# lcp29/trimesh-ray-optix

Hardware: AMD Instinct MI355X
Metric: Mrays/s closest-hit, 1M-tri mesh, 1024^2 ray batch (higher is better)
Workload: dtype f32; 1 GPU; C5(i): icosphere(8)+displacement seed 0, 1310720 tris; 1024x1024 pinhole rays per GPU; intersects_closest (stream_compaction=False); rays_per_gpu=1048576, rays_total=1048576, triangles=1310720, parallelism=ray-sharded x1, BVH replicated, warmup_steps_done=328, bvh_depth=30, bvh_bytes=104857568

## Files before the change

### trimesh-ray-optix_amd/csrc/kernels_direct.inc

```
template <bool C, bool DEEP = false> struct tr_word { typedef uint64_t T; };
template <> struct tr_word<true, false> { typedef uint32_t T; };

constexpr bool TR_STREAM_QN = true;
template <int Q> constexpr bool TR_STREAM_COLD = Q != TR_Q_CLOSEST;
template <int Q, int K, bool STATS, bool COMPACT = false, bool UNI = false, bool DEEP = false>
__device__ __forceinline__ void wave_traverse(const tr_bvh_view& b, tr_ray& r, bool go,
                                              tr_result& res, tr_topk<K>& top, tr_counters* cnt,
                                              const tr_ring ring) {
    tr_result_init(res);
    if (Q == TR_Q_LOCATION) top.init();
    typedef typename tr_word<COMPACT, DEEP>::T W;
    tr_state_t<W> fs;
    tr_state_init(fs);
    if (!go) fs.node = -1;
    while (!tr_done(fs)) {
        tr_fused_step<Q, K, STATS, COMPACT, W, UNI, true>(b, r, fs, res, top, cnt, ring);
        TR_CONVERGE();
        tr_fused_step<Q, K, STATS, COMPACT, W, UNI, false>(b, r, fs, res, top, cnt, ring);
        TR_CONVERGE();
    }
}

constexpr uint32_t TR_STEAL_EVERY = 3u;
constexpr uint32_t TR_STEAL_EARLY = 4u;
constexpr int TR_STEAL_IDLE = 1;
__device__ __forceinline__ int lane_rank(unsigned long long mask) {
    return (int)__builtin_amdgcn_mbcnt_hi((unsigned)(mask >> 32), __builtin_amdgcn_mbcnt_lo((unsigned)mask, 0u));
}

template <int Q, bool STATS, bool COMPACT, bool DEEP = false, bool QN = false>
__device__ __forceinline__ bool wave_traverse_steal(const tr_bvh_view& b, tr_ray& r, bool go,
                                                    tr_result& res, tr_counters* cnt,
                                                    const tr_ring ring, int32_t* wl, int lane,
                                                    uint32_t steal_min) {
    typedef typename tr_word<COMPACT, DEEP>::T W;
    tr_result_init(res);
    tr_topk<1> top;
    tr_state_t<W> fs;
    tr_state_init(fs);
    if (!go) fs.node = -1;
    auto trip_step = [&](auto test_tag) {
        constexpr bool TEST = decltype(test_tag)::value;
        if (!tr_done(fs)) tr_fused_step<Q, 1, STATS, COMPACT, W, false, TEST, QN>(b, r, fs, res, top, cnt, ring);
    };
    int owner = lane;
    bool split = false;
    uint32_t trip = 0;
    if (steal_min & 0x8000u) {
        steal_min &= 0x7fffu;
        const unsigned long long act = __ballot(go);
        if (act != 0ull) {
            const int l0 = (int)__builtin_ctzll(act);
            const float ax = __shfl(r.dx, l0), ay = __shfl(r.dy, l0), az = __shfl(r.dz, l0);
            const float bx = __shfl(r.ox, l0) - r.ox, by = __shfl(r.oy, l0) - r.oy, bz = __shfl(r.oz, l0) - r.oz;
            const float dd = ax * r.dx + ay * r.dy + az * r.dz;
            const float n0 = ax * ax + ay * ay + az * az, n1 = r.dx * r.dx + r.dy * r.dy + r.dz * r.dz;
            const float ex = 65535.f * b.frame.scale[0], ey = 65535.f * b.frame.scale[1], ez = 65535.f * b.frame.scale[2];
            const bool alike = dd > 0.f && dd * dd >= 0.998f * n0 * n1 && bx * bx + by * by + bz * bz <= 1e-4f * (ex * ex + ey * ey + ez * ez);
            if (4 * __popcll(__ballot(go && alike)) < 3 * __popcll(act) && steal_min > TR_STEAL_EARLY) steal_min = TR_STEAL_EARLY;
        }
    }
    typedef __attribute__((address_space(3))) volatile int32_t lds_i32;
    typedef __attribute__((address_space(3))) volatile unsigned long long lds_u64;
    lds_i32* const lw = (lds_i32*)wl;
    lds_i32* const list = lw;
    lds_i32* const xnode = lw + 64;
    lds_i32* const xdepth = lw + 128;
    constexpr int ACC = 192;
    int32_t* sum = wl + ACC;
    unsigned long long* keys = reinterpret_cast<unsigned long long*>(wl + ACC);
    lds_i32* const vsum = lw + ACC;
    lds_u64* const vkeys = (lds_u64*)(lw + ACC);
    lds_i32* const vslots = lw + ACC + 128;
    auto deposit = [&]() {
        if (Q == TR_Q_COUNT) {
            if (res.count) atomicAdd(&sum[owner], res.count);
        } else if (Q == TR_Q_ANY) {
            if (res.best_face >= 0) vsum[owner] = 1;
        } else {
            const bool have = res.best_slot >= 0;
            const unsigned long long key = ((unsigned long long)(__float_as_uint(res.best_t) & 0x7fffffffu) << 32) |
                                           (unsigned)res.best_face;
            if (have) atomicMin(&keys[owner], key);
            __builtin_amdgcn_wave_barrier();
            if (have && vkeys[owner] == key) vslots[owner] = res.best_slot;
        }
    };
    for (;;) {
#pragma unroll 1
        for (uint32_t k = 0; k <= TR_STEAL_EVERY; k += 2) {
            trip_step(std::true_type{});
            TR_CONVERGE();
            trip_step(std::false_type{});
            TR_CONVERGE();
        }
        trip += (TR_STEAL_EVERY / 2u + 1u) * 2u;
        if (split) {
            if (Q == TR_Q_ANY) {
                if (res.best_face >= 0) vsum[owner] = 1;
                __builtin_amdgcn_wave_barrier();
                if (vsum[owner] != 0 && !tr_done(fs)) { fs.node = -1; fs.p0 = -1; fs.p1 = -1; fs.p2 = -1; }
            } else if (Q == TR_Q_CLOSEST || Q == TR_Q_FIRST) {
                const bool have = res.best_slot >= 0;
                const unsigned long long mine = ((unsigned long long)(__float_as_uint(res.best_t) & 0x7fffffffu) << 32) |
                                                (unsigned)(res.best_face < 0 ? 0x7fffffff : res.best_face);
                if (have) atomicMin(&keys[owner], mine);
                __builtin_amdgcn_wave_barrier();
                const unsigned long long k = vkeys[owner];
                if (have && k == mine) vslots[owner] = res.best_slot;
                if (k < mine) {
                    tr_set_best_t(res, __uint_as_float((unsigned)(k >> 32)));
                    res.best_face = (int32_t)(unsigned)k;
                    res.best_slot = -1;
                }
            }
        }
        const bool done = tr_done(fs);
        const unsigned long long idle = __ballot(done);
        if (idle == ~0ull) break;
        if (__popcll(idle) >= TR_STEAL_IDLE) {
            const W cand = fs.trail & fs.owned;
            const bool can_give = !done && cand != 0 && trip >= steal_min;
            const unsigned long long donors = __ballot(can_give);
            const int ni = __popcll(idle), nd = __popcll(donors);
            const int np = ni < nd ? ni : nd;
            if (np > 0) {
                if (!split) {
                    if (Q == TR_Q_COUNT || Q == TR_Q_ANY) vsum[lane] = 0;
                    else vkeys[lane] = ~0ull;
                    split = true;
                    __builtin_amdgcn_wave_barrier();
                }
                const int drank = lane_rank(donors), irank = lane_rank(idle);
                const bool give = can_give && drank < np;
                int gnode = 0, gdepth = 0;
                if (give) {
                    uint32_t j;
                    gnode = tr_ring_get(ring, tr_bottom_slot<W>(fs.trail, fs.owned, j));
                    gdepth = (int32_t)(j + 1);
                    list[drank] = lane; xnode[lane] = gnode; xdepth[lane] = gdepth;
                    fs.trail &= ~(W(1) << j);
                }
                __builtin_amdgcn_wave_barrier();
                const bool take = done && irank < np;
                const int src = take ? list[irank] : lane;
                if (take) {
                    deposit();
                    tr_result_init(res);
                }
                r.ox = __shfl(r.ox, src); r.oy = __shfl(r.oy, src); r.oz = __shfl(r.oz, src);
                r.dx = __shfl(r.dx, src); r.dy = __shfl(r.dy, src); r.dz = __shfl(r.dz, src);
                r.ix = __shfl(r.ix, src); r.iy = __shfl(r.iy, src); r.iz = __shfl(r.iz, src);
                r.kd = __shfl(r.kd, src);
                r.sel_n = (uint32_t)__shfl((int)r.sel_n, src); r.sel_f = (uint32_t)__shfl((int)r.sel_f, src); r.sel_z = (uint32_t)__shfl((int)r.sel_z, src);
                if constexpr (QN) {
                    r.qax = __shfl(r.qax, src); r.qay = __shfl(r.qay, src); r.qaz = __shfl(r.qaz, src);
                    r.qnx = __shfl(r.qnx, src); r.qny = __shfl(r.qny, src); r.qnz = __shfl(r.qnz, src);
                    r.qfx = __shfl(r.qfx, src); r.qfy = __shfl(r.qfy, src); r.qfz = __shfl(r.qfz, src);
                    r.qaz2 = r.qaz;
                }
                const int own2 = __shfl(owner, src);
                const float bt = __shfl(res.best_t, src);
                if (take) {
                    owner = own2;
                    tr_state_init(fs);
                    fs.node = xnode[src];
                    fs.depth = (uint32_t)xdepth[src];
                    tr_set_best_t(res, bt);
                }
                __builtin_amdgcn_wave_barrier();
            }
        }
    }
    if (split) {
        deposit();
        __builtin_amdgcn_wave_barrier();
        if (Q == TR_Q_COUNT) {
            res.count = vsum[lane];
        } else if (Q == TR_Q_ANY) {
            res.best_face = vsum[lane] ? 0 : -1;
        } else {
            const unsigned long long k = vkeys[lane];
            tr_result_init(res);
            if (k != ~0ull) {
                tr_set_best_t(res, __uint_as_float((unsigned)(k >> 32)));
                res.best_face = (int32_t)(unsigned)k;
                res.best_slot = vslots[lane];
            }
        }
    }
    return split;
}

template <int Q, bool STATS, bool COMPACT = false, bool UNI = false, bool DEEP = false>
__device__ __forceinline__ void process_ray(const tr_bvh_view& b, const RayFetch& rf,
                                            const QueryOut& out, int64_t i, bool in_range,
                                            tr_counters* cnt, const tr_ring ring) {
    float o[3] = {0.f, 0.f, 0.f}, d[3] = {0.f, 0.f, 0.f};
    if (in_range) fetch_ray(rf, i, o, d);
    tr_ray r;
    const bool valid = tr_ray_setup_a(r, b.frame, o[0], o[1], o[2], d[0], d[1], d[2]) && in_range;
    tr_result res;
    if (Q == TR_Q_LOCATION) {
        tr_topk<0> top;
        top.ent = out.hits + (in_range ? i : 0) * out.cap;
        top.tris = b.tris;
        top.cap = out.cap;
        if (b.num_tris >= 2) {
            wave_traverse<Q, 0, STATS, COMPACT, UNI, DEEP>(b, r, valid, res, top, cnt, ring);
        } else {
            top.init();
            brute_one<Q>(b, r, valid, res);
            if (res.count) top.insert(res.best_t, res.best_face, 0);
        }
    } else {
        tr_topk<1> top;
        if (b.num_tris >= 2) wave_traverse<Q, 1, STATS, COMPACT, UNI, DEEP>(b, r, valid, res, top, cnt, ring);
        else brute_one<Q>(b, r, valid, res);
    }
    if (in_range) write_result<Q>(b, out, i, r, res);
}

template <int Q, bool STATS, bool COMPACT, bool DEEP = false, bool QN = false>
__device__ __forceinline__ void process_ray_steal(const tr_bvh_view& b, const RayFetch& rf,
                                                  const QueryOut& out, int64_t i, bool in_range,
                                                  tr_counters* cnt, const tr_ring ring, int32_t* wl,
                                                  uint32_t steal_min) {
    float o[3] = {0.f, 0.f, 0.f}, d[3] = {0.f, 0.f, 0.f};
    if (in_range) fetch_ray(rf, i, o, d);
    tr_ray r;
    const bool valid = tr_ray_setup_q(r, b.frame, o[0], o[1], o[2], d[0], d[1], d[2]) && in_range;
    tr_result res;
    bool split = false;
    if (b.num_tris >= 2) split = wave_traverse_steal<Q, STATS, COMPACT, DEEP, QN>(b, r, valid, res, cnt, ring, wl, (int)(threadIdx.x & 63), steal_min);
    else brute_one<Q>(b, r, valid, res);
    if (split && in_range) {
        fetch_ray(rf, i, o, d);
        tr_ray_setup_a(r, b.frame, o[0], o[1], o[2], d[0], d[1], d[2]);
    }
    if (in_range) write_result<Q>(b, out, i, r, res);
}

template <int Q, int K, bool STATS, bool COMPACT, bool DEEP = false>
__device__ __forceinline__ void wave_traverse_unordered(const tr_bvh_view& b, tr_ray& r, bool go,
                                                        tr_result& res, tr_topk<K>& top, tr_counters* cnt,
                                                        const tr_ring ring, const tr_leafq lq, int leaf_min) {
    typedef typename tr_word<COMPACT, DEEP>::T W;
    tr_result_init(res);
    if (Q == TR_Q_LOCATION) top.init();
    tr_ustate_t<W> st;
    tr_ustate_init(st);
    if (!go) st.node = -1;
    for (;;) {
        const bool can_node = tr_ucan_node(st);
        const unsigned long long mn = __ballot(can_node), ml = __ballot(st.nq > 0);
        if ((mn | ml) == 0ull) break;
        const bool parked = st.node >= 0 && !can_node;
        const bool leaf_phase = mn == 0ull || __ballot(parked) != 0ull || (int)__popcll(ml) >= (int)leaf_min;
        tr_unord_step<Q, K, STATS, COMPACT, W>(b, r, can_node, leaf_phase, st, res, top, cnt, ring, lq);
        TR_CONVERGE();
    }
}

template <int Q, bool STATS, bool COMPACT, bool DEEP = false>
__device__ __forceinline__ int wave_count_unordered_steal(const tr_bvh_view& b, tr_ray& r, bool go, tr_counters* cnt,
                                                          const tr_ring ring, const tr_leafq lq, int leaf_min,
                                                          int lane, uint32_t steal_min) {
    typedef typename tr_word<COMPACT, DEEP>::T W;
    tr_result res;
    tr_result_init(res);
    tr_topk<1> top;
    tr_ustate_t<W> st;
    tr_ustate_init(st);
    if (!go) st.node = -1;
    int owner = lane;
    int acc = 0;
    uint32_t trip = 0;
    auto hand_in = [&](bool want) {
        unsigned long long m = __ballot(want && res.count != 0);
        while (m != 0ull) {
            const int t = (int)__builtin_ctzll(m);
            const int o = __builtin_amdgcn_readlane(owner, t), c = __builtin_amdgcn_readlane(res.count, t);
            if (lane == o) acc += c;
            m &= m - 1ull;
        }
        if (want) res.count = 0;
    };
    for (;;) {
        bool live = true;
#pragma unroll 1
        for (int k = 0; k < 4 && live; k++) {
            const bool can_node = tr_ucan_node(st);
            const unsigned long long mn = __ballot(can_node), ml = __ballot(st.nq > 0);
            live = (mn | ml) != 0ull;
            if (live) {
                const bool parked = st.node >= 0 && !can_node;
                const bool leaf_phase = mn == 0ull || __ballot(parked) != 0ull || (int)__popcll(ml) >= (int)leaf_min;
                tr_unord_step<Q, 1, STATS, COMPACT, W>(b, r, can_node, leaf_phase, st, res, top, cnt, ring, lq);
            }
            TR_CONVERGE();
        }
        trip += 4;
        const bool done = tr_udone(st);
        const unsigned long long idle = __ballot(done);
        if (idle == ~0ull) break;
        if (idle == 0ull) continue;
        const W cand = st.trail & st.owned;
        const bool can_give = !done && cand != 0 && trip >= steal_min;
        const unsigned long long donors = __ballot(can_give);
        const int ni = __popcll(idle), nd = __popcll(donors);
        const int np = ni < nd ? ni : nd;
        if (np == 0) continue;
        const int drank = lane_rank(donors), irank = lane_rank(idle);
        const bool give = can_give && drank < np;
        const bool take = done && irank < np;
        const unsigned long long givers = __ballot(give);
        const int tgt = give ? drank : 63 - lane_rank(~givers);
        const int list = __builtin_amdgcn_ds_permute(tgt << 2, lane);
        const int pick = __shfl(list, irank & 63);
        const int src = take ? pick : lane;
        int gnode = 0, gdepth = 0;
// ... 145 lines not shown
        const uint32_t q = 255u - min(255u, (uint32_t)((float)cost[i] * scale));
        const int x = i < nfull ? (i / T) & 7 : i & 7;
        const uint32_t j = atomicAdd(&bins[x][q], 1u);
        const uint32_t sp = nsplit[x], q4 = sp >> 2;
        if (j < q4) {
            for (uint32_t k = 0; k < 4u; k++)
                order[(4u * j + k) * 8u + (uint32_t)x] = (uint32_t)i | (2u << 30) | (k << 28);
        } else if (j < sp) {
            const uint32_t p = 4u * q4 + 2u * (j - q4);
            order[p * 8u + (uint32_t)x] = (uint32_t)i | (1u << 30);
            order[(p + 1u) * 8u + (uint32_t)x] = (uint32_t)i | (1u << 30) | (1u << 28);
        } else {
            order[(j + sp + 2u * q4) * 8u + (uint32_t)x] = (uint32_t)i;
        }
        if (prev) prev[i] = cost[i];
        cost[i] = 0u;
    }
    if (tid == 0) { order[TR_SCHED_MAX] = (uint32_t)nblocks; order[TR_SCHED_MAX + 1] = (uint32_t)split; }
}

template <int Q, bool STATS, bool COMPACT, int BS, int MODE, bool DEEP, bool QN, bool JOB = false>
__device__ __forceinline__ void query_direct_body(const tr_bvh_view& b, const RayFetch& rf, const QueryOut& out,
                                                  int xcd_map, int scramble, int tile_w, int steal_min,
                                                  const uint32_t* __restrict__ order, int order_split,
                                                  uint32_t* __restrict__ cost,
                                                  unsigned long long* stats,
                                                  const int* __restrict__ sel,
                                                  const tr_wide_args& wa = tr_wide_args{nullptr, nullptr, 0, 0},
                                                  const tr_sort_job& job = tr_sort_job{nullptr, nullptr, nullptr, 0, 0, 0, 0, 0, 0}) {
    if (sel && *sel != 0) return;
    const unsigned slot_shift = JOB ? 8u : 0u;
    const unsigned bid = blockIdx.x - slot_shift;
    int64_t nblk = gridDim.x - slot_shift;
    const unsigned long long t_start = cost ? wall_clock64() : 0ull;
    __shared__ int32_t ring_lds[MODE == 4 ? 1 : TR_RING * BS];
    const tr_ring ring = {ring_lds + threadIdx.x, BS};
    constexpr int SCR = 384;
    __shared__ alignas(8) int32_t steal_lds[MODE == 1 ? (BS / 64) * SCR : (JOB ? 16 : 2)];
    if constexpr (JOB) {
        static_assert((MODE == 1 || MODE == 3) && BS == 128, "the sorter rides in the launches that steal");
        if (blockIdx.x < 8) {
            static_assert(sizeof(ring_lds) >= 8 * 256 * 4 && sizeof(steal_lds) >= 16 * 4, "the sorter works on the traversal's LDS");
            if (blockIdx.x == 0 && job.cost)
                sched_sort_body<BS>(job.cost, job.order, job.nblocks, job.xcd_map, job.split, job.split4, job.outlier8,
                                    job.floor_ticks, job.prev, reinterpret_cast<uint32_t(*)[256]>(ring_lds),
                                    reinterpret_cast<uint32_t*>(steal_lds));
            return;
        }
    }
    int64_t blk = bid;
    int part = 0, parts_lg = 0;
    if (order) {
        nblk -= 8 * ((int64_t)order_split + 2 * (order_split >> 2));
        const uint32_t* hdr = order + TR_SCHED_MAX;
        if (hdr[0] != (uint32_t)nblk || hdr[1] != (uint32_t)order_split) {
            order = nullptr;
            if ((int64_t)bid >= nblk) return;
        }
    }
    if (order) {
        const uint32_t e = order[bid];
        blk = e & 0x07ffffffu;
        if (blk >= nblk) return;
        parts_lg = (int)(e >> 30);
        part = (int)((e >> 28) & 3u);
        if (MODE != 1 && MODE != 3) {
            if (part) return;
            parts_lg = 0;
        }
    } else if (xcd_map > 0) {
        const int64_t T = xcd_map, span = 8 * T;
        const int64_t nfull = nblk / span * span;
        if (blk < nfull) {
            const int64_t x = blk & 7;
            int64_t k = blk >> 3;
            if (scramble > 1) k = (k * scramble) % (nfull >> 3);
            blk = ((k / T) * 8 + x) * T + (k % T);
        }
    }
    int64_t i = blk * BS + threadIdx.x;
    if (tile_w > 0) {
        const int lgh = (tile_w >> 28) & 3, lgw = 6 - lgh;
        const int64_t width = tile_w & 0x0fffffff;
        const int64_t tile = i >> 6, tpr = width >> lgw;
        const int lane = (int)(i & 63);
        const int64_t ty = tile / tpr, tx = tile - ty * tpr;
        i = ((ty << lgh) + (lane >> lgw)) * width + (tx << lgw) + (lane & ((1 << lgw) - 1));
    }
    tr_counters cnt = {0, 0, 0};
    if (MODE == 4) {
        __shared__ int32_t wstack_lds[(TR_WNODES + TR_WLEAVES) * BS];
        const bool in_range = i < rf.n;
        float o[3] = {0.f, 0.f, 0.f}, d[3] = {0.f, 0.f, 0.f};
        if (in_range) fetch_ray(rf, i, o, d);
        tr_ray r;
        const bool valid = tr_ray_setup_q(r, b.frame, o[0], o[1], o[2], d[0], d[1], d[2]) && in_range;
        tr_result res;
        if constexpr (Q == TR_Q_LOCATION) {
            tr_topk<0> top;
            top.ent = out.hits + (in_range ? i : 0) * out.cap;
            top.tris = b.tris;
            top.cap = out.cap;
            wave_traverse_wide<Q, 0, STATS, BS>(b, wa, r, valid, res, top, cnt, wstack_lds);
        } else {
            tr_topk<1> top;
            wave_traverse_wide<Q, 1, STATS, BS>(b, wa, r, valid, res, top, cnt, wstack_lds);
        }
        if (in_range) write_result<Q>(b, out, i, r, res);
    } else if (MODE == 2) {
        __shared__ int32_t leafq_lds[TR_LEAFQ * BS];
        const tr_leafq lq = {leafq_lds + threadIdx.x, BS};
        process_ray_unordered<Q, STATS, COMPACT, DEEP>(b, rf, out, i, i < rf.n, &cnt, ring, lq, steal_min);
    } else if (MODE == 3) {
        __shared__ int32_t leafq_lds[TR_LEAFQ * BS];
        const tr_leafq lq = {leafq_lds + threadIdx.x, BS};
        const bool mine = (((int)threadIdx.x ^ part) & ((1 << parts_lg) - 1)) == 0;
        const uint32_t smin = parts_lg ? ((uint32_t)steal_min >> 20) & 0xfffu : ((uint32_t)steal_min >> 8) & 0xfffu;
        process_ray_unordered<Q, STATS, COMPACT, DEEP, true>(b, rf, out, i, i < rf.n && mine, &cnt, ring, lq,
                                                            steal_min & 0xff, smin);
    } else if (MODE == 1) {
        const bool mine = (((int)threadIdx.x ^ part) & ((1 << parts_lg) - 1)) == 0;
        const uint32_t smin = parts_lg ? (uint32_t)steal_min >> 16 : (uint32_t)steal_min & 0xffffu;
        process_ray_steal<Q, STATS, COMPACT, DEEP, QN>(b, rf, out, i, i < rf.n && mine, &cnt, ring,
                                                       steal_lds + (threadIdx.x >> 6) * SCR, smin);
    } else {
        process_ray<Q, STATS, COMPACT, !STATS && BS == 128 && Q != TR_Q_LOCATION, DEEP>(b, rf, out, i, i < rf.n, &cnt, ring);
    }
    if (cost && (threadIdx.x & 63) == 0) {
        constexpr int TR_SPLIT_STICKY = 1;
        const unsigned long long dt = (wall_clock64() - t_start) << (parts_lg ? parts_lg + TR_SPLIT_STICKY : 0);
        atomicMax(&cost[blk], (uint32_t)(dt > 0x7ffffull ? 0x7ffffull : dt));
    }
    flush_stats<STATS>(cnt, stats);
}

#ifndef TR_DIRECT_WAVES
#define TR_DIRECT_WAVES 6
#endif
#if TR_DIRECT_WAVES > 0
#ifndef TR_DEEP_WAVES
#define TR_DEEP_WAVES TR_DIRECT_WAVES
#endif
#define TR_DIRECT_W ((!COMPACT || (DEEP && !QN)) ? TR_DEEP_WAVES - 1 : DEEP ? TR_DEEP_WAVES : TR_DIRECT_WAVES)
#define TR_DIRECT_OCC __attribute__((amdgpu_waves_per_eu(TR_DIRECT_W, TR_DIRECT_W)))
#else
#define TR_DIRECT_OCC
#endif
constexpr int TR_BS = 128;
template <int Q, bool STATS, bool COMPACT, int MODE = 0, bool DEEP = false, bool QN = false>
__global__ __launch_bounds__(TR_BS) TR_DIRECT_OCC void k_query_direct(tr_bvh_view b, RayFetch rf, QueryOut out,
                                                      int xcd_map, int scramble, int tile_w, int steal_min,
                                                      const uint32_t* __restrict__ order, int order_split,
                                                      uint32_t* __restrict__ cost,
                                                      unsigned long long* stats,
                                                      const int* __restrict__ sel) {
    TR_VIEW_LIVE(b);
    query_direct_body<Q, STATS, COMPACT, TR_BS, MODE, DEEP, QN>(b, rf, out, xcd_map, scramble, tile_w, steal_min, order,
                                                                order_split, cost, stats, sel);
}
#ifndef TR_COUNT_WAVES
#define TR_COUNT_WAVES 7
#endif
#if TR_COUNT_WAVES > 0
#define TR_COUNT_W ((DEEP || !COMPACT) ? 5 : TR_COUNT_WAVES)
#define TR_COUNT_OCC __attribute__((amdgpu_waves_per_eu(TR_COUNT_W, TR_COUNT_W)))
#else
#define TR_COUNT_OCC
#endif
template <bool COMPACT, bool DEEP>
__global__ __launch_bounds__(TR_BS) TR_COUNT_OCC void k_query_count_steal(tr_bvh_view b, RayFetch rf, QueryOut out,
// ... 91 lines not shown
```

### trimesh-ray-optix_amd/csrc/tr_bvh.h

```cpp
#pragma once
#include <type_traits>
#include "tr_math.h"
#include "../../include/triro_hip.h"

struct alignas(16) tr_f4 {
    float x, y, z, w;
};
struct alignas(16) tr_i4 {
    int32_t x, y, z, w;
};

struct alignas(64) tr_node {
    float box0[6];
    float box1[6];
    int32_t c0, c1;
    int32_t parent;
    int32_t sibling;
};
static_assert(sizeof(tr_node) == 64, "node must be 64 B");
TR_HD void tr_node_set_box(float* box, const float* lo, const float* hi) {
    box[0] = lo[0]; box[1] = lo[1]; box[2] = lo[2]; box[3] = hi[2]; box[4] = hi[0]; box[5] = hi[1];
}

struct alignas(8) tr_link {
// ... 278 lines not shown
#endif
                const tr_tri u = tr_load_tri<false, COMPACT>(b, pe, nc);
                if (!tr_tie_own(r.dx, r.dy, r.dz, u.ax, u.ay, u.az, u.bx, u.by, u.bz, u.cx, u.cy, u.cz, e.tie)) tt = -1.0f;
            }
            const bool hit = tt >= TR_TMIN && tt <= TR_TMAX;
            fin = tr_fold_hit<Q, K>(hit, tt, t.face, pe, res, top);
            pe = -1;
        }
    }
    return fin;
}

#define TR_RING 16
struct tr_ring {
    int32_t* base;
    int32_t stride;
};
TR_HD int32_t tr_ring_get(const tr_ring& ring, uint32_t slot) {
#if defined(__HIP_DEVICE_COMPILE__)
    typedef __attribute__((address_space(3))) int32_t tr_lds_i32;
    return ((tr_lds_i32*)ring.base)[slot * ring.stride];
#else
    return ring.base[slot * ring.stride];
#endif
}
TR_HD void tr_ring_put(const tr_ring& ring, uint32_t slot, int32_t v) {
#if defined(__HIP_DEVICE_COMPILE__)
    typedef __attribute__((address_space(3))) int32_t tr_lds_i32;
    ((tr_lds_i32*)ring.base)[slot * ring.stride] = v;
#else
    ring.base[slot * ring.stride] = v;
#endif
}

template <typename W>
struct tr_state_t {
    int32_t node;
    uint32_t depth;
    W trail;
    W owned;
    int32_t p0, p1, p2;
    int32_t pe;
};
typedef tr_state_t<uint64_t> tr_state;
typedef tr_state_t<uint32_t> tr_state32;

TR_HD uint32_t tr_top_bit(uint64_t x) { return 63u - (uint32_t)__builtin_clzll(x); }
TR_HD uint32_t tr_top_bit(uint32_t x) { return 31u - (uint32_t)__builtin_clz(x); }
TR_HD uint64_t tr_ring_mask(uint64_t) { return 0x0001000100010001ull; }
TR_HD uint32_t tr_ring_mask(uint32_t) { return 0x00010001u; }
TR_HD uint32_t tr_popc(uint64_t x) { return (uint32_t)__builtin_popcountll(x); }
TR_HD uint32_t tr_popc(uint32_t x) { return (uint32_t)__builtin_popcount(x); }

template <typename W>
TR_HD void tr_push_far(const tr_ring ring, W trail, W& owned, uint32_t depth, int32_t node) {
    if (ring.base && tr_popc(owned & trail) < TR_RING) {
        tr_ring_put(ring, tr_popc(owned) & (TR_RING - 1), node);
        owned |= W(1) << depth;
    }
}
template <typename W>
TR_HD bool tr_pop_far(const tr_ring ring, W& trail, W& owned, uint32_t& j, int32_t& node) {
    j = tr_top_bit(trail);
    const W bit = W(1) << j;
    trail &= ~bit;
    const bool own = (owned & bit) != 0;
    owned &= bit - 1;
    if (!(ring.base && own)) return false;
    node = tr_ring_get(ring, tr_popc(owned) & (TR_RING - 1));
    return true;
}
template <typename W>
TR_HD uint32_t tr_bottom_slot(W trail, W owned, uint32_t& j) {
    j = (uint32_t)__builtin_ctzll((unsigned long long)(trail & owned));
    return tr_popc((W)(owned & ((W(1) << j) - 1))) & (TR_RING - 1);
}

template <typename W>
TR_HD void tr_state_init(tr_state_t<W>& st) {
    st.node = 0; st.depth = 0; st.trail = 0; st.owned = 0;
    st.p0 = -1; st.p1 = -1; st.p2 = -1; st.pe = -1;
}

template <typename W>
TR_HD bool tr_pending(const tr_state_t<W>& st) { return st.p0 >= 0 || st.p1 >= 0; }
template <typename W>
TR_HD bool tr_done(const tr_state_t<W>& st) { return st.node < 0 && st.p0 < 0 && st.p1 < 0 && st.pe < 0; }

TR_HD void tr_node_slabs(const tr_ray& r, const tr_f4& n0, const tr_f4& n1, const tr_f4& n2,
                         float& tn0, float& tf0, float& tn1, float& tf1) {
#if defined(__HIP_DEVICE_COMPILE__)
    typedef float tr_v2 __attribute__((ext_vector_type(2)));
    const tr_v2 oxy = {r.ox, r.oy}, ozz = {r.oz, r.oz};
    const tr_v2 ixy = {r.ix, r.iy}, izz = {r.iz, r.iz};
    const tr_v2 a = (tr_v2{n0.x, n0.y} - oxy) * ixy;
    const tr_v2 b = (tr_v2{n0.z, n0.w} - ozz) * izz;
    const tr_v2 c = (tr_v2{n1.x, n1.y} - oxy) * ixy;
    const tr_v2 d = (tr_v2{n1.z, n1.w} - oxy) * ixy;
    const tr_v2 e = (tr_v2{n2.x, n2.y} - ozz) * izz;
    const tr_v2 f = (tr_v2{n2.z, n2.w} - oxy) * ixy;
    tn0 = fmaxf(fmaxf(fminf(a.x, c.x), fminf(a.y, c.y)), fminf(b.x, b.y));
    tf0 = fminf(fminf(fmaxf(a.x, c.x), fmaxf(a.y, c.y)), fmaxf(b.x, b.y)) * TR_SLAB_PAD;
    tn1 = fmaxf(fmaxf(fminf(d.x, f.x), fminf(d.y, f.y)), fminf(e.x, e.y));
    tf1 = fminf(fminf(fmaxf(d.x, f.x), fmaxf(d.y, f.y)), fmaxf(e.x, e.y)) * TR_SLAB_PAD;
#else
    tr_slab(r, n0.x, n0.y, n0.z, n1.x, n1.y, n0.w, tn0, tf0);
    tr_slab(r, n1.z, n1.w, n2.x, n2.z, n2.w, n2.y, tn1, tf1);
#endif
}

template <int Q, bool STATS>
TR_HD void tr_node_step(const tr_bvh_view& b, const tr_ray& r, tr_state& st, const tr_result& res,
                        tr_counters* cnt, const tr_ring ring) {
    const tr_f4* np = reinterpret_cast<const tr_f4*>(b.nodes + st.node);
    const tr_f4 n0 = np[0], n1 = np[1], n2 = np[2], n3 = np[3];
    if (STATS) cnt->nodes++;
    float tn0, tf0, tn1, tf1;
    tr_node_slabs(r, n0, n1, n2, tn0, tf0, tn1, tf1);
    union { float f; int32_t i; } u0, u1, u2, u3;
    u0.f = n3.x; u1.f = n3.y; u2.f = n3.z; u3.f = n3.w;
    const int32_t c0 = u0.i, c1 = u1.i;
    int32_t parent = u2.i, sibling = u3.i;
    const float lim = tr_cull_limit<Q>(res);
    bool h0 = tr_slab_hit(tn0, tf0, lim);
    bool h1 = tr_slab_hit(tn1, tf1, lim);
    if (h0 && c0 < 0) { st.p0 = ~c0; h0 = false; }
    if (h1 && c1 < 0) { st.p1 = ~c1; h1 = false; }
    if (h0 | h1) {
        const bool both = h0 & h1;
        const bool swap = both ? (tn1 < tn0) : h1;
        if (both) {
            tr_push_far(ring, st.trail, st.owned, st.depth, swap ? c0 : c1);
            st.trail |= (1ull << st.depth);
        }
        st.node = swap ? c1 : c0;
        st.depth++;
    } else if (st.trail == 0) {
        st.node = -1;
    } else {
        uint32_t j = 0;
        int32_t far = -1;
        if (tr_pop_far(ring, st.trail, st.owned, j, far)) {
            st.node = far;
        } else {
            int32_t node = st.node;
            uint32_t depth = st.depth;
            while (depth > j + 1) {
                node = parent;
                const tr_link l = b.links[node];
                parent = l.parent; sibling = l.sibling;
                depth--;
                if (STATS) cnt->climbs++;
            }
            st.node = sibling;
        }
        st.depth = j + 1;
    }
}

template <int Q, int K, bool STATS>
TR_HD void tr_leaf_step(const tr_bvh_view& b, const tr_ray& r, tr_state& st, tr_result& res,
                        tr_topk<K>& top, tr_counters* cnt) {
    const int32_t q0 = st.p0, q1 = st.p1;
    tr_counters* nc = nullptr;
    const bool any1 = TR_WAVE_ANY(q1 >= 0);
    const tr_tri t0 = tr_load_tri<false>(b, q0 >= 0 ? q0 : 0, nc);
// ... 70 lines not shown
#endif
}

template <bool STATS>
TR_HD int32_t tr_climb(const tr_bvh_view& b, int32_t node, uint32_t depth, uint32_t j, tr_counters* cnt) {
    tr_link l = b.links[node];
    if (STATS) cnt->climbs++;
    while (depth > j + 1) {
        node = l.parent;
        l = b.links[node];
        depth--;
        if (STATS) cnt->climbs++;
    }
    return l.sibling;
}

struct tr_rec_f { tr_f4 n0, n1, n2, n3; };
struct tr_rec_q { tr_i4 w0, w1; };
TR_HD void tr_rec_slabs(const tr_bvh_view&, const tr_ray& r, const tr_rec_f& n, float& tn0, float& tf0, float& tn1, float& tf1) {
    tr_node_slabs(r, n.n0, n.n1, n.n2, tn0, tf0, tn1, tf1);
}
TR_HD void tr_rec_slabs(const tr_bvh_view& b, const tr_ray& r, const tr_rec_q& n, float& tn0, float& tf0, float& tn1, float& tf1) {
    tr_qnode_slabs(r, b.frame, n.w0, n.w1, tn0, tf0, tn1, tf1);
}
TR_HD void tr_rec_children(const tr_rec_f& n, int32_t& c0, int32_t& c1) {
    union { float f; int32_t i; } u0, u1;
    u0.f = n.n3.x; u1.f = n.n3.y; c0 = u0.i; c1 = u1.i;
}
TR_HD void tr_rec_children(const tr_rec_q& n, int32_t& c0, int32_t& c1) { c0 = n.w1.z; c1 = n.w1.w; }
TR_HD void tr_rec_links(const tr_rec_f& n, int32_t& parent, int32_t& sibling) {
    union { float f; int32_t i; } u2, u3;
    u2.f = n.n3.z; u3.f = n.n3.w; parent = u2.i; sibling = u3.i;
}
TR_HD void tr_rec_links(const tr_rec_q&, int32_t& parent, int32_t& sibling) { parent = -1; sibling = -1; }

template <int Q, int K, bool STATS, bool COMPACT, typename W, bool TEST, bool COLD, typename REC>
TR_HD void tr_fused_body(const tr_bvh_view& b, const tr_ray& r, tr_state_t<W>& st, tr_result& res,
                         tr_topk<K>& top, tr_counters* cnt, const tr_ring ring, const bool has_node,
                         const REC& rec) {
    if (STATS && has_node) cnt->nodes++;
    bool fin = false;
    const int32_t q0 = st.p0;
    if (TEST && TR_WAVE_ANY(q0 >= 0)) {
        tr_counters* nc = nullptr;
        const tr_tri t0 = tr_load_tri<false, COMPACT>(b, q0 >= 0 ? q0 : 0, nc);
        const bool live = q0 >= 0;
        if (STATS && live) cnt->tris++;
        fin = tr_fold_leaf<Q, K>(live, r, t0, q0, res, top, st.pe);
    }
    if (Q == TR_Q_ANY && fin) { st.node = -1; st.p1 = -1; st.p2 = -1; }
    float tn0, tf0, tn1, tf1;
    tr_rec_slabs(b, r, rec, tn0, tf0, tn1, tf1);
    int32_t c0, c1, parent, sibling;
    tr_rec_children(rec, c0, c1);
    tr_rec_links(rec, parent, sibling);
    const float lim = tr_cull_limit<Q>(res);
    const bool go = has_node && st.node >= 0;
    bool h0 = tr_slab_hit(tn0, tf0, lim) && go;
    bool h1 = tr_slab_hit(tn1, tf1, lim) && go;
    if (!TEST) {
        const bool l0 = h0 && c0 < 0, l1 = h1 && c1 < 0;
        h0 = h0 && c0 >= 0;
        h1 = h1 && c1 >= 0;
        if (go) {
            const bool hb = st.p0 >= 0, two = l0 && l1;
            const int32_t xi = l0 ? ~c0 : (l1 ? ~c1 : -1);
            st.p2 = (hb && two) ? ~c1 : -1;
            st.p1 = hb ? xi : (two ? ~c1 : -1);
            st.p0 = hb ? st.p0 : xi;
        }
    } else {
        const bool l0 = h0 && c0 < 0;
        const bool wait = st.p2 >= 0;
        const bool l1 = (h1 && c1 < 0) || wait;
        h0 = h0 && c0 >= 0;
        h1 = h1 && c1 >= 0;
        const int32_t i1 = wait ? st.p2 : ~c1;
        const bool hb = st.p1 >= 0, two = l0 && l1;
        const int32_t xi = l0 ? ~c0 : (l1 ? i1 : -1);
        st.p0 = hb ? st.p1 : xi;
        st.p1 = hb ? xi : (two ? i1 : -1);
        st.p2 = (hb && two) ? i1 : -1;
    }
    if (go) {
        if (h0 || h1) {
            const bool both = h0 && h1;
            const bool swap = (both && tn1 < tn0) || !h0;
            if (both) {
                tr_push_far(ring, st.trail, st.owned, st.depth, swap ? c0 : c1);
                st.trail |= (W(1) << st.depth);
            }
            st.node = swap ? c1 : c0;
            st.depth++;
        } else if (st.trail == 0) {
            st.node = -1;
        } else {
            uint32_t j = 0;
            int32_t far = -1;
            if (!tr_pop_far(ring, st.trail, st.owned, j, far)) {
                if constexpr (std::is_same<REC, tr_rec_f>::value) {
                    int32_t node = st.node;
                    uint32_t depth = st.depth;
                    while (depth > j + 1) {
                        node = parent;
                        const tr_link l = b.links[node];
                        parent = l.parent; sibling = l.sibling;
                        depth--;
                        if (STATS) cnt->climbs++;
                    }
                    far = sibling;
                } else {
                    far = tr_climb<STATS>(b, st.node, st.depth, j, cnt);
                }
            }
            st.node = far;
            st.depth = j + 1;
        }
    }
    if (TEST) {
        if (tr_drain_exact<Q, K, COMPACT, COLD>(b, r, st.pe, res, top) && Q == TR_Q_ANY) { st.node = -1; st.p0 = -1; st.p1 = -1; st.p2 = -1; }
        st.pe = -1;
    }
}


template <int Q, int K, bool STATS, bool COMPACT = false, typename W = uint64_t, bool UNI = false, bool TEST = true,
          bool QN = false, bool COLD = true>
TR_HD void tr_fused_step(const tr_bvh_view& b, const tr_ray& r, tr_state_t<W>& st, tr_result& res,
                         tr_topk<K>& top, tr_counters* cnt, const tr_ring ring) {
    const int32_t room = TEST ? st.p2 : st.p1;
    const bool has_node = st.node >= 0 && room < 0;
#if defined(__HIP_DEVICE_COMPILE__)
    if (UNI) {
        const unsigned long long m = __ballot(has_node);
        if (m != 0ull) {
            const int32_t nu = __builtin_amdgcn_readlane(st.node, (int)__builtin_ctzll(m));
            if (__ballot(has_node && st.node != nu) == 0ull) {
                if constexpr (QN) {
                    typedef const __attribute__((address_space(4))) tr_i4* tr_ci4p;
                    const tr_ci4p sp = (tr_ci4p)(unsigned long long)tr_qnode_ptr<COMPACT>(b, nu);
                    const tr_rec_q rec = {sp[0], sp[1]};
                    tr_fused_body<Q, K, STATS, COMPACT, W, TEST, COLD>(b, r, st, res, top, cnt, ring, has_node, rec);
                } else {
                    typedef const __attribute__((address_space(4))) tr_f4* tr_cf4p;
                    const tr_cf4p sp = (tr_cf4p)(unsigned long long)tr_node_ptr<COMPACT>(b, nu);
                    const tr_rec_f rec = {sp[0], sp[1], sp[2], sp[3]};
                    tr_fused_body<Q, K, STATS, COMPACT, W, TEST, COLD>(b, r, st, res, top, cnt, ring, has_node, rec);
                }
                return;
            }
        }
    }
#endif
    const int32_t nidx = st.node & ~(st.node >> 31) & (room >> 31);
    if constexpr (QN) {
        const tr_i4* np = tr_qnode_ptr<COMPACT>(b, nidx);
        const tr_rec_q rec = {np[0], np[1]};
        tr_fused_body<Q, K, STATS, COMPACT, W, TEST, COLD>(b, r, st, res, top, cnt, ring, has_node, rec);
    } else {
        const tr_f4* np = tr_node_ptr<COMPACT>(b, nidx);
        const tr_rec_f rec = {np[0], np[1], np[2], np[3]};
        tr_fused_body<Q, K, STATS, COMPACT, W, TEST, COLD>(b, r, st, res, top, cnt, ring, has_node, rec);
    }
}


constexpr int TR_LEAFQ = 6;
// ... 12 lines not shown
};

template <typename W>
TR_HD void tr_ustate_init(tr_ustate_t<W>& st) { st.node = 0; st.depth = 0; st.trail = 0; st.owned = 0; st.nq = 0; st.pe = -1; }
template <typename W>
TR_HD bool tr_udone(const tr_ustate_t<W>& st) { return st.node < 0 && st.nq == 0 && st.pe < 0; }
template <typename W>
TR_HD bool tr_ucan_node(const tr_ustate_t<W>& st) { return st.node >= 0 && st.nq <= TR_LEAFQ - 2; }

template <int Q, int K, bool STATS, bool COMPACT, typename W>
TR_HD void tr_unord_step(const tr_bvh_view& b, const tr_ray& r, bool go_node, bool leaf_phase,
                         tr_ustate_t<W>& st, tr_result& res, tr_topk<K>& top, tr_counters* cnt,
                         const tr_ring ring, const tr_leafq lq) {
    const int32_t nidx = go_node ? st.node : 0;
    const tr_i4* np = COMPACT ? reinterpret_cast<const tr_i4*>(reinterpret_cast<const char*>(b.qnodes) + ((uint32_t)nidx << 5))
                              : reinterpret_cast<const tr_i4*>(b.qnodes + nidx);
    const tr_i4 w0 = np[0], w1 = np[1];
    if (STATS && go_node) cnt->nodes++;
    bool fin = false;
    if (leaf_phase) {
        const bool gl = st.nq > 0;
        int32_t slot = 0;
        if (gl) { st.nq--; slot = lq.base[st.nq * lq.stride]; }
        tr_counters* nc = nullptr;
        const tr_tri t = tr_load_tri<false, COMPACT>(b, slot, nc);
        if (STATS && gl) cnt->tris++;
        fin = tr_fold_leaf<Q, K>(gl, r, t, slot, res, top, st.pe);
    }
    if (Q == TR_Q_ANY && fin) { st.node = -1; st.nq = 0; }
    const bool go = go_node && !fin;
    float tn0, tf0, tn1, tf1;
    tr_qnode_slabs(r, b.frame, w0, w1, tn0, tf0, tn1, tf1);
    const int32_t c0 = w1.z, c1 = w1.w;
    bool h0 = tr_slab_hit(tn0, tf0, TR_TLIM) && go;
    bool h1 = tr_slab_hit(tn1, tf1, TR_TLIM) && go;
    if (h0 && c0 < 0) { lq.base[st.nq * lq.stride] = ~c0; st.nq++; h0 = false; }
    if (h1 && c1 < 0) { lq.base[st.nq * lq.stride] = ~c1; st.nq++; h1 = false; }
    if (go) {
        if (h0 || h1) {
            const bool both = h0 && h1;
            const bool swap = (Q == TR_Q_ANY) ? ((both && tn1 < tn0) || !h0) : !h0;
            if (both) {
                st.trail |= (W(1) << st.depth);
                if (ring.base) {
                    const uint32_t slot = st.depth & (TR_RING - 1);
                    tr_ring_put(ring, slot, swap ? c0 : c1);
                    st.owned = (st.owned & ~(tr_ring_mask(W(0)) << slot)) | (W(1) << st.depth);
                }
            }
            st.node = swap ? c1 : c0;
            st.depth++;
        } else if (st.trail == 0) {
            st.node = -1;
        } else {
            const uint32_t j = tr_top_bit(st.trail);
            st.trail &= ~(W(1) << j);
            if (ring.base && ((st.owned >> j) & W(1))) st.node = tr_ring_get(ring, j & (TR_RING - 1));
            else st.node = tr_climb<STATS>(b, st.node, st.depth, j, cnt);
            st.depth = j + 1;
        }
    }
    if (leaf_phase) {
        if (tr_drain_exact<Q, K, COMPACT>(b, r, st.pe, res, top) && Q == TR_Q_ANY) { st.node = -1; st.nq = 0; }
        st.pe = -1;
    }
}

template <int Q, int K, bool STATS>
TR_HD void tr_traverse_unordered(const tr_bvh_view& b, const tr_ray& r, bool valid, tr_result& res,
                                 tr_topk<K>& top, tr_counters* cnt, const tr_ring ring, const tr_leafq lq) {
    tr_result_init(res);
    if (Q == TR_Q_LOCATION) top.init();
    if (!valid || b.num_tris < 2) return;
    tr_ustate_t<uint64_t> st;
    tr_ustate_init(st);
    while (!tr_udone(st)) {
        const bool cn = tr_ucan_node(st);
        tr_unord_step<Q, K, STATS, false, uint64_t>(b, r, cn, !cn, st, res, top, cnt, ring, lq);
        TR_CONVERGE();
    }
}

template <int Q, int K, bool STATS>
TR_HD void tr_traverse(const tr_bvh_view& b, const tr_ray& r, bool valid, tr_result& res,
                       tr_topk<K>& top, tr_counters* cnt, const tr_ring ring = tr_ring{nullptr, 0}) {
    tr_result_init(res);
    if (Q == TR_Q_LOCATION) top.init();
    if (!valid || b.num_tris < 2) return;
    tr_state st;
    tr_state_init(st);
    while (!tr_done(st)) {
        if (tr_pending(st)) tr_leaf_step<Q, K, STATS>(b, r, st, res, top, cnt);
        else tr_node_step<Q, STATS>(b, r, st, res, cnt, ring);
        TR_CONVERGE();
    }
}
```

Before: 7121 Mrays/s.

## Add plain-stack traversal state for quantized steal path with overflow retraversal fallback

When QN is set, the work-stealing traversal uses a simple stack pointer with ring push/pop in place of the trail/owned bitmask restart scheme. Stealing gives away the bottom stack entry, and stack overflow sets a lost flag so the ray is retraversed with a full-stack fallback. This aims to cut the bitmask bookkeeping and the restart-from-root cost on pops. The tile index computation is also changed to use a wave-uniform block and wave id. The risk is extra LDS flag traffic, and rays that overflow the ring pay a slow noinline retraversal.

Result: faster. 7553 Mrays/s (median of 6 runs) (+6.1%).

```diff
diff --git a/trimesh-ray-optix_amd/csrc/kernels_direct.inc b/trimesh-ray-optix_amd/csrc/kernels_direct.inc
--- a/trimesh-ray-optix_amd/csrc/kernels_direct.inc
+++ b/trimesh-ray-optix_amd/csrc/kernels_direct.inc
@@ -32,8 +32,10 @@
 __device__ __forceinline__ bool wave_traverse_steal(const tr_bvh_view& b, tr_ray& r, bool go,
                                                     tr_result& res, tr_counters* cnt,
                                                     const tr_ring ring, int32_t* wl, int lane,
-                                                    uint32_t steal_min) {
-    typedef typename tr_word<COMPACT, DEEP>::T W;
+                                                    uint32_t steal_min, bool& lost) {
+    constexpr bool PLAIN = QN;
+    typedef typename std::conditional<PLAIN, tr_plain_w, typename tr_word<COMPACT, DEEP>::T>::type W;
+    lost = false;
     tr_result_init(res);
     tr_topk<1> top;
     tr_state_t<W> fs;
@@ -66,6 +68,8 @@
     lds_i32* const list = lw;
     lds_i32* const xnode = lw + 64;
     lds_i32* const xdepth = lw + 128;
+    int32_t* const xflags = wl + 128;
+    if constexpr (PLAIN) xdepth[lane] = 0;
     constexpr int ACC = 192;
     int32_t* sum = wl + ACC;
     unsigned long long* keys = reinterpret_cast<unsigned long long*>(wl + ACC);
@@ -73,6 +77,9 @@
     lds_u64* const vkeys = (lds_u64*)(lw + ACC);
     lds_i32* const vslots = lw + ACC + 128;
     auto deposit = [&]() {
+        if constexpr (PLAIN) {
+            if (tr_plain_lost(fs.sp)) atomicOr(&xflags[owner], 0x100);
+        }
         if (Q == TR_Q_COUNT) {
             if (res.count) atomicAdd(&sum[owner], res.count);
         } else if (Q == TR_Q_ANY) {
@@ -119,8 +126,15 @@
         const unsigned long long idle = __ballot(done);
         if (idle == ~0ull) break;
         if (__popcll(idle) >= TR_STEAL_IDLE) {
-            const W cand = fs.trail & fs.owned;
-            const bool can_give = !done && cand != 0 && trip >= steal_min;
+            uint32_t bot = 0;
+            bool has_far;
+            if constexpr (PLAIN) {
+                bot = (uint32_t)xdepth[lane] & 0xffu;
+                has_far = tr_plain_can_give(fs.sp, bot);
+            } else {
+                has_far = (fs.trail & fs.owned) != 0;
+            }
+            const bool can_give = !done && has_far && trip >= steal_min;
             const unsigned long long donors = __ballot(can_give);
             const int ni = __popcll(idle), nd = __popcll(donors);
             const int np = ni < nd ? ni : nd;
@@ -134,7 +148,14 @@
                 const int drank = lane_rank(donors), irank = lane_rank(idle);
                 const bool give = can_give && drank < np;
                 int gnode = 0, gdepth = 0;
-                if (give) {
+                (void)gdepth;
+                if constexpr (PLAIN) {
+                    if (give) {
+                        gnode = tr_plain_give(ring, bot);
+                        list[drank] = lane; xnode[lane] = gnode;
+                        atomicAdd(&xflags[lane], 1);
+                    }
+                } else if (give) {
                     uint32_t j;
                     gnode = tr_ring_get(ring, tr_bottom_slot<W>(fs.trail, fs.owned, j));
                     gdepth = (int32_t)(j + 1);
@@ -165,7 +186,8 @@
                     owner = own2;
                     tr_state_init(fs);
                     fs.node = xnode[src];
-                    fs.depth = (uint32_t)xdepth[src];
+                    if constexpr (PLAIN) atomicAnd(&xflags[lane], 0x100);
+                    else fs.depth = (uint32_t)xdepth[src];
                     tr_set_best_t(res, bt);
                 }
                 __builtin_amdgcn_wave_barrier();
@@ -188,6 +210,9 @@
                 res.best_slot = vslots[lane];
             }
         }
+        if constexpr (PLAIN) lost = (xdepth[lane] & 0x100) != 0;
+    } else if constexpr (PLAIN) {
+        lost = tr_plain_lost(fs.sp);
     }
     return split;
 }
@@ -221,6 +246,26 @@
     if (in_range) write_result<Q>(b, out, i, r, res);
 }
 
+template <int Q>
+__device__ __attribute__((noinline)) tr_result retraverse_lost(const tr_node* nodes, const tr_link* links, const tr_tri* tris,
+                                                               float b0, float b1, float b2, float s0, float s1, float s2,
+                                                               float ox, float oy, float oz, float dx, float dy, float dz,
+                                                               float best_t, int32_t best_face, int32_t best_slot) {
+    tr_bvh_view v;
+    v.nodes = nodes; v.links = links; v.tris = tris; v.num_tris = 2; v.qnodes = nullptr; v.frame_dev = nullptr;
+    v.frame.base[0] = b0; v.frame.base[1] = b1; v.frame.base[2] = b2;
+    v.frame.scale[0] = s0; v.frame.scale[1] = s1; v.frame.scale[2] = s2;
+    tr_result res;
+    res.best_t = best_t; res.best_face = best_face; res.best_slot = best_slot; res.count = 0;
+    tr_ray r;
+    if (tr_ray_setup_a(r, v.frame, ox, oy, oz, dx, dy, dz)) {
+        tr_topk<1> top;
+        tr_counters* nc = nullptr;
+        tr_traverse_more<Q, 1, false>(v, r, res, top, nc);
+    }
+    return res;
+}
+
 template <int Q, bool STATS, bool COMPACT, bool DEEP = false, bool QN = false>
 __device__ __forceinline__ void process_ray_steal(const tr_bvh_view& b, const RayFetch& rf,
                                                   const QueryOut& out, int64_t i, bool in_range,
@@ -231,12 +276,23 @@
     tr_ray r;
     const bool valid = tr_ray_setup_q(r, b.frame, o[0], o[1], o[2], d[0], d[1], d[2]) && in_range;
     tr_result res;
-    bool split = false;
-    if (b.num_tris >= 2) split = wave_traverse_steal<Q, STATS, COMPACT, DEEP, QN>(b, r, valid, res, cnt, ring, wl, (int)(threadIdx.x & 63), steal_min);
+    bool split = false, lost = false;
+    if (b.num_tris >= 2) split = wave_traverse_steal<Q, STATS, COMPACT, DEEP, QN>(b, r, valid, res, cnt, ring, wl, (int)(threadIdx.x & 63), steal_min, lost);
     else brute_one<Q>(b, r, valid, res);
     if (split && in_range) {
         fetch_ray(rf, i, o, d);
         tr_ray_setup_a(r, b.frame, o[0], o[1], o[2], d[0], d[1], d[2]);
+    }
+    if constexpr (QN) {
+        lost = lost && valid;
+        if (__builtin_expect(TR_WAVE_ANY(lost), 0)) {
+            if (lost) {
+                fetch_ray(rf, i, o, d);
+                res = retraverse_lost<Q>(b.nodes, b.links, b.tris, b.frame.base[0], b.frame.base[1], b.frame.base[2],
+                                         b.frame.scale[0], b.frame.scale[1], b.frame.scale[2], o[0], o[1], o[2], d[0], d[1], d[2],
+                                         res.best_t, res.best_face, res.best_slot);
+            }
+        }
     }
     if (in_range) write_result<Q>(b, out, i, r, res);
 }
@@ -548,10 +604,12 @@
     if (tile_w > 0) {
         const int lgh = (tile_w >> 28) & 3, lgw = 6 - lgh;
         const int64_t width = tile_w & 0x0fffffff;
-        const int64_t tile = i >> 6, tpr = width >> lgw;
-        const int lane = (int)(i & 63);
-        const int64_t ty = tile / tpr, tx = tile - ty * tpr;
-        i = ((ty << lgh) + (lane >> lgw)) * width + (tx << lgw) + (lane & ((1 << lgw) - 1));
+        static_assert(BS % 64 == 0, "a wave is one tile");
+        const uint32_t wave = (uint32_t)__builtin_amdgcn_readfirstlane((int)(threadIdx.x >> 6));
+        const uint32_t tile = (uint32_t)blk * (uint32_t)(BS / 64) + wave, tpr = (uint32_t)(width >> lgw);
+        const int lane = (int)(threadIdx.x & 63);
+        const uint32_t ty = tile / tpr, tx = tile - ty * tpr;
+        i = (((int64_t)ty << lgh) + (lane >> lgw)) * width + ((int64_t)tx << lgw) + (lane & ((1 << lgw) - 1));
     }
     tr_counters cnt = {0, 0, 0};
     if (MODE == 4) {
diff --git a/trimesh-ray-optix_amd/csrc/tr_bvh.h b/trimesh-ray-optix_amd/csrc/tr_bvh.h
--- a/trimesh-ray-optix_amd/csrc/tr_bvh.h
+++ b/trimesh-ray-optix_amd/csrc/tr_bvh.h
@@ -384,6 +384,41 @@
     st.p0 = -1; st.p1 = -1; st.p2 = -1; st.pe = -1;
 }
 
+struct tr_plain_w {};
+template <>
+struct tr_state_t<tr_plain_w> {
+    int32_t node;
+    uint32_t sp;
+    int32_t p0, p1, p2;
+    int32_t pe;
+};
+typedef tr_state_t<tr_plain_w> tr_pstate;
+TR_HD void tr_state_init(tr_pstate& st) {
+    st.node = 0; st.sp = 0;
+    st.p0 = -1; st.p1 = -1; st.p2 = -1; st.pe = -1;
+}
+TR_HD void tr_plain_push(const tr_ring ring, uint32_t& sp, int32_t node) {
+    if (sp < 2u * TR_RING) {
+        tr_ring_put(ring, sp >> 1, node);
+        sp += 2u;
+    } else {
+        sp |= 1u;
+    }
+}
+TR_HD int32_t tr_plain_pop(const tr_ring ring, uint32_t& sp) {
+    if (sp < 2u) return -1;
+    sp -= 2u;
+    return tr_ring_get(ring, sp >> 1);
+}
+TR_HD bool tr_plain_lost(uint32_t sp) { return (sp & 1u) != 0; }
+TR_HD bool tr_plain_can_give(uint32_t sp, uint32_t bot) { return (sp >> 1) > bot; }
+TR_HD int32_t tr_plain_give(const tr_ring ring, uint32_t& bot) {
+    const int32_t node = tr_ring_get(ring, bot);
+    tr_ring_put(ring, bot, -1);
+    bot++;
+    return node;
+}
+
 template <typename W>
 TR_HD bool tr_pending(const tr_state_t<W>& st) { return st.p0 >= 0 || st.p1 >= 0; }
 template <typename W>
@@ -620,7 +655,18 @@
         st.p1 = hb ? xi : (two ? i1 : -1);
         st.p2 = (hb && two) ? i1 : -1;
     }
-    if (go) {
+    if constexpr (std::is_same<W, tr_plain_w>::value) {
+        if (go) {
+            if (h0 || h1) {
+                const bool both = h0 && h1;
+                const bool swap = (both && tn1 < tn0) || !h0;
+                if (both) tr_plain_push(ring, st.sp, swap ? c0 : c1);
+                st.node = swap ? c1 : c0;
+            } else {
+                st.node = tr_plain_pop(ring, st.sp);
+            }
+        }
+    } else if (go) {
         if (h0 || h1) {
             const bool both = h0 && h1;
             const bool swap = (both && tn1 < tn0) || !h0;
@@ -799,6 +845,18 @@
 }
 
 template <int Q, int K, bool STATS>
+TR_HD void tr_traverse_more(const tr_bvh_view& b, const tr_ray& r, tr_result& res, tr_topk<K>& top, tr_counters* cnt) {
+    if (Q == TR_Q_ANY && res.best_face >= 0) return;
+    tr_state st;
+    tr_state_init(st);
+    while (!tr_done(st)) {
+        if (tr_pending(st)) tr_leaf_step<Q, K, STATS>(b, r, st, res, top, cnt);
+        else tr_node_step<Q, STATS>(b, r, st, res, cnt, tr_ring{nullptr, 0});
+        TR_CONVERGE();
+    }
+}
+
+template <int Q, int K, bool STATS>
 TR_HD void tr_traverse(const tr_bvh_view& b, const tr_ray& r, bool valid, tr_result& res,
                        tr_topk<K>& top, tr_counters* cnt, const tr_ring ring = tr_ring{nullptr, 0}) {
     tr_result_init(res);
```
